# AIGC-Audio/AudioGPT

Hardware: NVIDIA H100
Metric: mel_frames_per_s_vocoded (higher is better)
Workload: dtype f32

## Files before the change

### audiogpt_b200/csrc/tapconv.cuh

```cuda
#pragma once
#include <cuda_fp16.h>
#include "common.cuh"

namespace agpt {

constexpr int kMaxTaps = 12;
constexpr int TC_BM = 128;
constexpr int TC_KC = 8;

enum Pro : int { PRO_NONE = 0, PRO_LRELU = 1, PRO_ADDVEC = 2, PRO_SILU = 3 };
enum Epi : int {
  EPI_BIAS = 0,
  EPI_RES = 1,
  EPI_ACC = 2,
  EPI_RELU = 3,
  EPI_ADDVEC = 4,
  EPI_GATE = 5,
  EPI_GEGLU = 6,
  EPI_DIFFOUT = 7,
  EPI_STORE_CF = 8,
  EPI_TANH = 9,
  EPI_MISH = 10,
  EPI_SILU = 11,
  EPI_GELU_SCALED = 12,
};

struct TapConvParams {
  const float* in; long in_gstride; int in_pitch;
  const float* w;
  const float* bias;
  float* out; long out_gstride; int out_pitch;
  int G, L, Wreal, Cin, cin_pad, Cout, cout_pad;
  int ntaps; int tap_off[kMaxTaps];
  int lo_al, R;
  int pro; float slope; const float* pvec; int pvec_gstride;
  int epi; const float* res; long res_gstride; int res_pitch; float scale; int accumulate;
  const float* evec; int evec_gstride;
  float* out2; long out2_gstride; int out2_pitch; int csplit;
  const float* w_h; const float* w_h256; const float* w_h64; const float* w_h96; int tc_chunks_h; float tc_descale;
  int tc_bn, tc_na, tc_nw, tc_nr, tc_nwk, tc_nb, tc_tps, tc_flags, tc_flags_user;
  long long* dbg;
  float flops_scale;
  int strips, strip_w;
  __half* pl_hi; __half* pl_lo; int pl_pitch;
  int tc_tall;
  const __half* pi_hi; const __half* pi_lo;
  __half* po_hi; __half* po_lo; float po_slope;
  int tc_dual;
  int tc_pipe;
  int tc_narrow_pipe;
  int tc_conv_pipe;
};

__host__ __device__ inline int tc_wv(const TapConvParams& P) { return P.Wreal > 0 ? (P.strips > 0 ? P.strip_w + 2 : P.Wreal + 1) : 0; }
__host__ __device__ inline int tc_lv(const TapConvParams& P) { const int wv = tc_wv(P); return wv ? (P.L / P.Wreal) * wv : P.L; }
__host__ __device__ inline int tc_groups(const TapConvParams& P) { return P.strips > 0 ? P.G * P.strips : P.G; }
__host__ __device__ inline int tc_sample(const TapConvParams& P, int gz) { return P.strips > 0 ? gz / P.strips : gz; }
__host__ __device__ inline int tc_row_in(const TapConvParams& P, int gz, int q, int Wv, int Lv) {
  if (q < 0 || q >= Lv) return -1;
  if (!Wv) return q;
  const int h = q / Wv, j = q - h * Wv;
  if (P.strips > 0) {
    const int w = (gz % P.strips) * P.strip_w + j - 1;
    return (w >= 0 && w < P.Wreal) ? h * P.Wreal + w : -1;
  }
  return j < P.Wreal ? h * P.Wreal + j : -1;
}
__host__ __device__ inline int tc_row_out(const TapConvParams& P, int gz, int q, int Wv, int Lv) {
  if (q < 0 || q >= Lv) return -1;
  if (!Wv) return q;
  const int h = q / Wv, j = q - h * Wv;
  if (P.strips > 0) {
    if (j < 1 || j > P.strip_w) return -1;
    const int w = (gz % P.strips) * P.strip_w + j - 1;
    return w < P.Wreal ? h * P.Wreal + w : -1;
  }
  return j < P.Wreal ? h * P.Wreal + j : -1;
}


struct PackedConv {
  DevBuf w, b, w_h, w_h256, w_h64, w_h96;
  int tc_bn = 0, h_chunks = 0;
  float h_descale = 1.f;
  int Cin = 0, cin_pad = 0, Cout = 0, cout_pad = 0, ntaps = 0;
  int tap_off_1d[kMaxTaps] = {0};
  bool is2d = false;
  bool has_bias = false;
  float useful = 1.f;
};

inline int tc_pick_bn(int cout) {
  if (cout <= 32) return 32;
  if (cout <= 64) return 64;
  const int w128 = round_up(cout, 128), w64 = round_up(cout, 64);
  return (w128 <= w64) ? 128 : 64;
}

struct PackedConv;
void tapconv_launch(TapConvParams P, cudaStream_t st);
void tcconv_launch(TapConvParams P, cudaStream_t st);
bool tcconv5_launch(TapConvParams P, cudaStream_t st);
bool tcpair_launch(TapConvParams c1, TapConvParams c2, cudaStream_t st);
struct HTile { int bn; const float* w; long ntiles; int mt; };
HTile pick_h_tile(const TapConvParams& P, int sms);
void pack_h_weights(struct PackedConv& pc, const std::vector<float>& h);
bool tcconv_supported(const TapConvParams& P);
void pack_tc_weights(struct PackedConv& pc, const std::vector<float>& h);
void tc_set_enabled(int on);
bool tc_enabled();
void profile_enable(int on);
void* profile_begin(const TapConvParams& P, bool tc, double bytes_override, cudaStream_t st);
void* profile_begin_pair(const TapConvParams& c1, const TapConvParams& c2, cudaStream_t st);
void profile_end(void* rec, cudaStream_t st);
void profile_count_tall();
long long profile_tall_launches();
void profile_count_dual();
long long profile_dual_launches();
void profile_count_pipe();
long long profile_pipe_launches();
void profile_count_narrow_pipe();
long long profile_narrow_pipe_launches();
void profile_count_conv_pipe();
long long profile_conv_pipe_launches();
void profile_count_plane();
long long profile_plane_launches();
void tapconv_note_launch(int tc, int bn, int mt, int plane);
void tapconv_last_launch(int ran[4]);
void plane_split(const float* x, __half* hi, __half* lo, long n, float slope, cudaStream_t st);
void profile_collect(double* ms, double* flops, double* bytes, long long* launches);
long profile_dump(char* out, long cap);
double fma_peak_tflops();

inline TapConvParams tapconv_params(const PackedConv& pc, int G, int L, int Wreal, int dil) {
  TapConvParams P;
  memset(&P, 0, sizeof(P));
  P.w = pc.w.p;
  P.bias = pc.has_bias ? pc.b.p : nullptr;
  P.G = G; P.L = L; P.Wreal = Wreal;
  P.Cin = pc.Cin; P.cin_pad = pc.cin_pad; P.Cout = pc.Cout; P.cout_pad = pc.cout_pad;
  P.ntaps = pc.ntaps;
  if (pc.is2d) {
    AGPT_CHECK(pc.ntaps == 9 && Wreal > 0, "2d conv needs W");
    const int Wv = Wreal + 1;
    for (int dh = -1, t = 0; dh <= 1; ++dh)
      for (int dw = -1; dw <= 1; ++dw, ++t) P.tap_off[t] = dh * Wv + dw;
  } else {
    for (int t = 0; t < pc.ntaps; ++t) P.tap_off[t] = pc.tap_off_1d[t] * dil;
  }
  P.scale = 1.f;
  P.flops_scale = pc.useful;
  P.tc_bn = pc.tc_bn;
  P.w_h = pc.w_h.p; P.w_h256 = pc.w_h256.p; P.w_h64 = pc.w_h64.p; P.w_h96 = pc.w_h96.p; P.tc_chunks_h = pc.h_chunks; P.tc_descale = pc.h_descale;
  return P;
}

inline void tapconv_set_strips(TapConvParams& P, int strip_w) {
  AGPT_CHECK(P.Wreal > 0 && P.ntaps == 9 && strip_w >= 8, "strip mode is for 3x3 convs");
  P.strips = cdiv(P.Wreal, strip_w);
  P.strip_w = strip_w;
  const int Wv = strip_w + 2;
  for (int dh = -1, t = 0; dh <= 1; ++dh)
    for (int dw = -1; dw <= 1; ++dw, ++t) P.tap_off[t] = dh * Wv + dw;
}

inline void pack_conv(PackedConv& pc, const float* w, const float* b, int Cout, int Cin, int K, bool is2d,
                      float wscale = 1.f) {
  pc.Cin = Cin; pc.Cout = Cout; pc.cin_pad = round_up(Cin, TC_KC); pc.cout_pad = round_up(Cout, 32);
  pc.ntaps = K; pc.is2d = is2d;
  std::vector<float> h((size_t)K * pc.cin_pad * pc.cout_pad, 0.f);
  for (int co = 0; co < Cout; ++co)
    for (int ci = 0; ci < Cin; ++ci)
      for (int k = 0; k < K; ++k)
        h[((size_t)k * pc.cin_pad + ci) * pc.cout_pad + co] = w[((size_t)co * Cin + ci) * K + k] * wscale;
  pc.w.upload(h);
  pack_tc_weights(pc, h);
  if (!is2d) {
    const int c = (K - 1) / 2;
    for (int k = 0; k < K; ++k) pc.tap_off_1d[k] = k - c;
  }
  pc.has_bias = b != nullptr;
  std::vector<float> hb(pc.cout_pad, 0.f);
  if (b) for (int co = 0; co < Cout; ++co) hb[co] = b[co];
  pc.b.upload(hb);
}

inline void pack_conv_grouped(PackedConv& pc, const float* w, const float* b, int C, int K, int g) {
  const int c = (K - 1) / 2;
  auto fdiv = [](int a, int d) { return a >= 0 ? a / d : -((-a + d - 1) / d); };
  const int smin = fdiv(-c, g), smax = fdiv(g - 1 + K - 1 - c, g);
  const int nt = smax - smin + 1;
  AGPT_CHECK(nt <= kMaxTaps, "grouped conv: too many super-taps");
  const int Cg = g * C;
  std::vector<float> wg((size_t)Cg * Cg * nt, 0.f), bg(Cg, 0.f);
  for (int j = 0; j < g; ++j)
    for (int co = 0; co < C; ++co) {
      if (b) bg[j * C + co] = b[co];
      for (int i = 0; i < g; ++i)
        for (int ci = 0; ci < C; ++ci)
          for (int s = smin; s <= smax; ++s) {
            const int t = g * s + i - j + c;
            if (t < 0 || t >= K) continue;
            wg[((size_t)(j * C + co) * Cg + (i * C + ci)) * nt + (s - smin)] = w[((size_t)co * C + ci) * K + t];
          }
    }
  pack_conv(pc, wg.data(), b ? bg.data() : nullptr, Cg, Cg, nt, false);
// ... 50 lines not shown
```

### audiogpt_b200/csrc/tcconv5.cu

```cuda
#include "tapconv.cuh"
#include "tapconv_epi.cuh"
#include "tc_common.cuh"
#include "tc_h16.cuh"
#include "tc_tma.cuh"
#include "models.h"

namespace agpt {

namespace {

constexpr int MAX_NA = 4, MAX_NW = 8;
constexpr int kMaxDyn = 227 * 1024 - 256;
constexpr int kDualDyn = 113 * 1024 - 256;

struct Tc5Smem {
  uint32_t a_hi[MAX_NA], a_lo[MAX_NA], w[MAX_NW], raw[2], rowinfo, rowp, bars, total;
};
__host__ __device__ inline void tc5_layout(Tc5Smem& s, int BN, int MT, int RRA, int NA, int NW, int NR, bool pl = false,
                                           int raw_pitch = 256) {
  uint32_t o = 0;
  for (int i = 0; i < MAX_NA; ++i) { s.a_hi[i] = o; if (i < NA) o += RRA * 128; }
  for (int i = 0; i < MAX_NA; ++i) { s.a_lo[i] = o; if (i < NA) o += RRA * 128; }
  for (int i = 0; i < MAX_NW; ++i) { s.w[i] = o; if (i < NW) o += 2 * BN * 128; }
  for (int i = 0; i < 2; ++i) { s.raw[i] = o; if (i < NR) o += RRA * raw_pitch; }
// ... 621 lines not shown
      if ((MT == TC_TALL || HALF) && blk == 0) load_block(0);
      named_bar_sync(1, NWK);
      const int jc = xt & 7;
      const float4 cv = epi_colvec(P2, g, cb + 4 * jc);
#pragma unroll
      for (int i = 0; i < 8; ++i) {
        const int idx = xt + i * NWK;
        const int row = (idx >> 3) & (MT - 1);
        if (pp[i] >= 0)
          epi_store_cv<PL>(P2, g, pp[i], cb + 4 * jc, *reinterpret_cast<const float4*>(stg + sw128(row, jc)), pre[i], cv);
        if (i + LA < nitem) {
          const int idxa = idx + LA * NWK;
          pp[i + LA] = rowp[item_row(xt, i + LA)];
          if (pp[i + LA] >= 0) epi_load(P2, g, pp[i + LA], cb + 4 * (idxa & 7), pre[i + LA]);
        }
      }
      if (cb + 32 < BN) load_block(cb + 32);
    }
  } else if (lane == 0) {
    const uint32_t bytes = 2u * BN * 128u;
    const int total2 = P2.tc_chunks_h * P2.ntaps;
    for (int it = 0; it < total + total2; ++it) {
      if constexpr (PL)
        if (it < total && it % P1.ntaps == 0) pl_load_chunk(smem, S, tmh, tml, a_full, a_empty, NA, it / P1.ntaps, qa + lo, g, RRA);
      const int s = it % NW, n = it / NW;
      if (n >= 1) mbar_wait(&w_empty[s], (uint32_t)((n - 1) & 1));
      mbar_arrive_expect_tx(&w_full[s], bytes);
      const uint8_t* src = it < total ? reinterpret_cast<const uint8_t*>(P1.w_h) + (size_t)it * bytes
                                      : reinterpret_cast<const uint8_t*>(P2.w_h) + (size_t)(it - total) * bytes;
      bulk_g2s(smem + S.w[s], src, bytes, &w_full[s]);
    }
  }
}

template <int BN, int MT>
__global__ void __launch_bounds__(V5_THREADS, 1) tcpair_kernel(const __grid_constant__ TapConvParams P1,
                                                               const __grid_constant__ TapConvParams P2) {
  tcpair_body<BN, MT, false>(P1, P2, nullptr, nullptr);
}
template <int BN>
__global__ void __launch_bounds__(V5_THREADS, 2) tcpair2_kernel(const __grid_constant__ TapConvParams P1,
                                                                const __grid_constant__ TapConvParams P2) {
  tcpair_body<BN, TC_ROWS, false, true>(P1, P2, nullptr, nullptr);
}
template <int BN, int MT>
__global__ void __launch_bounds__(V5_THREADS, 1) tcpair_pl_kernel(const __grid_constant__ TapConvParams P1,
                                                                 const __grid_constant__ TapConvParams P2,
                                                                 const __grid_constant__ CUtensorMap tmh,
                                                                 const __grid_constant__ CUtensorMap tml) {
  tcpair_body<BN, MT, true>(P1, P2, &tmh, &tml);
}

constexpr int PIPE_THREADS = 512;
constexpr int PIPE_MMA = 256, PIPE_DATA = 128;
template <int N> __device__ __forceinline__ void setmaxnreg_inc() { asm volatile("setmaxnreg.inc.sync.aligned.u32 %0;" ::"n"(N)); }
template <int N> __device__ __forceinline__ void setmaxnreg_dec() { asm volatile("setmaxnreg.dec.sync.aligned.u32 %0;" ::"n"(N)); }

struct PipeSmem { uint32_t set[2], w[MAX_NW], bars, total; };
__host__ __device__ inline void pipe_layout(PipeSmem& s, int R1, int NW) {
  uint32_t o = 0;
  for (int i = 0; i < 2; ++i) { s.set[i] = o; o += (uint32_t)R1 * 512; }
  for (int i = 0; i < MAX_NW; ++i) { s.w[i] = o; if (i < NW) o += 2 * 128 * 128; }
  s.bars = o; o += (2 * MAX_NW + 4) * 8;
  s.total = o;
}

__global__ void __launch_bounds__(PIPE_THREADS, 1) tcpair_pipe_kernel(const __grid_constant__ TapConvParams P1,
                                                                      const __grid_constant__ TapConvParams P2) {
  constexpr int BN = 128, MT = TC_ROWS;
  extern __shared__ uint8_t smem_raw_[];
  uint8_t* smem = reinterpret_cast<uint8_t*>((reinterpret_cast<uintptr_t>(smem_raw_) + 1023) & ~(uintptr_t)1023);
  const int R1 = P1.R, NW = P1.tc_nw;
  __shared__ PipeSmem S;
  if (threadIdx.x == 0) pipe_layout(S, R1, NW);
  __syncthreads();
  uint64_t* w_full = reinterpret_cast<uint64_t*>(smem + S.bars);
  uint64_t* w_empty = w_full + MAX_NW;
  uint64_t* in_full = w_full + 2 * MAX_NW;
  uint64_t* acc_full = in_full + 2;

  const int tid = threadIdx.x, warp = tid >> 5, lane = tid & 31;
  const int wg = __shfl_sync(0xffffffffu, tid >> 7, 0);
  int span2 = 0;
  for (int t = 0; t < P2.ntaps; ++t) span2 = max(span2, P2.tap_off[t] - P2.lo_al);
  const int Lv = P1.L, MTO = MT - span2, ntx = (Lv + MTO - 1) / MTO, ntiles = ntx * P1.G;
  const int nloc = (int)blockIdx.x < ntiles ? (ntiles - 1 - (int)blockIdx.x) / (int)gridDim.x + 1 : 0;
  const int lo = P1.lo_al, nch = P1.tc_chunks_h, total1 = nch * P1.ntaps;
  const int RR2 = P2.R, nch2 = P2.tc_chunks_h, total2 = nch2 * P2.ntaps;
  auto tile_of = [&](int k, int& g, int& q0) {
    const int T = (int)blockIdx.x + k * (int)gridDim.x;
    g = T / ntx;
    q0 = (T - g * ntx) * MTO;
  };

  if (tid == 0) {
    for (int i = 0; i < NW; ++i) { mbar_init(&w_full[i], 1); mbar_init(&w_empty[i], PIPE_MMA / 32); }
    for (int i = 0; i < 2; ++i) { mbar_init(&in_full[i], PIPE_DATA); mbar_init(&acc_full[i], PIPE_MMA); }
    fence_barrier_init();
  }
  __syncthreads();
  pdl_wait();

  if (wg < 2) {
    setmaxnreg_inc<168>();
    float acc[BN / 2];
    int it = 0, prev = -1;
    auto mma_taps = [&](const TapConvParams& Q, uint32_t ahi0, uint32_t alo0, int ksteps) {
      for (int t = 0; t < Q.ntaps; ++t, ++it) {
        const int s = it % NW;
        mbar_wait(&w_full[s], (uint32_t)((it / NW) & 1));
        const uint32_t shift = (uint32_t)Q.tap_off[t] * 128u;
        const uint64_t dah = make_desc(ahi0 + shift), dal = make_desc(alo0 + shift);
        const uint32_t ws = smem_u32(smem + S.w[s]);
        fence_acc<BN / 2>(acc);
        wgmma_fence();
        for (int k = 0; k < ksteps; ++k) {
          const uint64_t ko = (uint64_t)((k * 32) >> 4);
          const uint64_t dwh = make_desc(ws) + ko, dwl = make_desc(ws + BN * 128) + ko;
          wgmma_n128(acc, dah + ko, dwh);
          wgmma_n128(acc, dal + ko, dwh);
          wgmma_n128(acc, dah + ko, dwl);
        }
        wgmma_commit();
        wgmma_wait<1>();
        fence_acc<BN / 2>(acc);
        if (prev >= 0 && lane == 0) mbar_arrive(&w_empty[prev]);
        prev = s;
      }
    };
    auto drain = [&]() {
      wgmma_wait<0>();
      fence_acc<BN / 2>(acc);
      if (prev >= 0 && lane == 0) mbar_arrive(&w_empty[prev]);
      prev = -1;
    };
    const int r0 = wg * (MT / 2) + (warp & 3) * 16 + (lane >> 2), c0 = 2 * (lane & 3);
    for (int k = 0; k < nloc; ++k) {
      int g, q0;
      tile_of(k, g, q0);
      const int qa = q0 + P2.lo_al;
      uint8_t* set = smem + S.set[k & 1];
#pragma unroll
      for (int i = 0; i < BN / 2; ++i) acc[i] = 0.f;
      mbar_wait(&in_full[k & 1], (uint32_t)((k >> 1) & 1));
      for (int c = 0; c < nch; ++c) {
        const uint32_t ahi0 = smem_u32(set) + (uint32_t)c * R1 * 128 + (uint32_t)(wg * (MT / 2) - lo) * 128u;
        mma_taps(P1, ahi0, ahi0 + (uint32_t)nch * R1 * 128, (min(H_KCH, P1.Cin - c * H_KCH) + 15) >> 4);
      }
      drain();
      named_bar_sync(1, PIPE_MMA);
      const uint32_t lo_part = (uint32_t)nch2 * RR2 * 128;
      const float dsc1 = P1.tc_descale;
#pragma unroll
      for (int i = 0; i < BN / 8; ++i) {
        const int col = 8 * i + c0;
        const bool cok = col < P2.Cin;
        float2 bv = make_float2(0.f, 0.f);
        if (cok && P1.bias) bv = __ldg(reinterpret_cast<const float2*>(P1.bias + col));
        uint8_t* hi = set + (uint32_t)(col >> 6) * RR2 * 128;
#pragma unroll
        for (int h = 0; h < 2; ++h) {
          const int r = r0 + 8 * h;
          float v0 = 0.f, v1 = 0.f;
          if (cok && qa + r >= 0 && qa + r < Lv) {
            v0 = lrelu(__fadd_rn(__fmul_rn(acc[4 * i + 2 * h], dsc1), bv.x), P2.slope);
            v1 = lrelu(__fadd_rn(__fmul_rn(acc[4 * i + 2 * h + 1], dsc1), bv.y), P2.slope);
          }
          uint32_t l;
          const uint32_t hw = split2(v0, v1, l);
          const uint32_t o = sw128(r, (col & 63) >> 3) + (col & 7) * 2;
          *reinterpret_cast<uint32_t*>(hi + o) = hw;
          *reinterpret_cast<uint32_t*>(hi + lo_part + o) = l;
        }
      }
      const int zitems = (RR2 - MT) * 8;
      for (int idx = tid; idx < zitems * 2 * nch2; idx += PIPE_MMA) {
        const int blk = idx / zitems, u = idx - blk * zitems;
        *reinterpret_cast<uint4*>(set + (uint32_t)blk * RR2 * 128 + MT * 128 + u * 16) = make_uint4(0u, 0u, 0u, 0u);
      }
#pragma unroll
      for (int i = 0; i < BN / 2; ++i) acc[i] = 0.f;
      fence_proxy_async();
      named_bar_sync(1, PIPE_MMA);
      for (int c = 0; c < nch2; ++c) {
        const uint32_t ahi0 = smem_u32(set) + (uint32_t)c * RR2 * 128 + (uint32_t)(wg * (MT / 2) - P2.lo_al) * 128u;
        mma_taps(P2, ahi0, ahi0 + lo_part, (min(H_KCH, P2.Cin - c * H_KCH) + 15) >> 4);
      }
      drain();
      named_bar_sync(1, PIPE_MMA);
      const float dsc = P2.tc_descale;
#pragma unroll
      for (int blk = 0; blk < BN / 32; ++blk) {
        uint8_t* stg = set + blk * (MT * 128);
        const float* a = &acc[4 * (blk * 32 / 8)];
#pragma unroll
        for (int i8 = 0; i8 < 4; ++i8) {
          const int col = 8 * i8 + c0;
          *reinterpret_cast<float2*>(stg + sw128(r0, col >> 2) + (col & 3) * 4) = make_float2(a[4 * i8] * dsc, a[4 * i8 + 1] * dsc);
          *reinterpret_cast<float2*>(stg + sw128(r0 + 8, col >> 2) + (col & 3) * 4) =
              make_float2(a[4 * i8 + 2] * dsc, a[4 * i8 + 3] * dsc);
        }
      }
      mbar_arrive(&acc_full[k & 1]);
    }
  } else if (wg == 2) {
    setmaxnreg_inc<152>();
    const int dt = tid - PIPE_MMA;
    auto transform = [&](int k) {
      int g, q0;
      tile_of(k, g, q0);
      const int rin = q0 + P2.lo_al + lo;
      const float* __restrict__ ing = P1.in + g * P1.in_gstride;
      uint8_t* set = smem + S.set[k & 1];
      const int items = R1 * nch * 8;
#pragma unroll 4
      for (int idx = dt; idx < items; idx += PIPE_DATA) {
        const int row = idx / (nch * 8), c = (idx >> 3) % nch, q = idx & 7;
        const int r = rin + row, ch = c * H_KCH + 8 * q;
        float4 v0 = make_float4(0.f, 0.f, 0.f, 0.f), v1 = v0;
        if (r >= 0 && r < Lv && ch < P1.Cin) {
          v0 = ldg_stream(ing + (long)r * P1.in_pitch + ch);
          v1 = ldg_stream(ing + (long)r * P1.in_pitch + ch + 4);
        }
        const float4 x0 = pro_apply5(P1, v0, true, nullptr), x1 = pro_apply5(P1, v1, true, nullptr);
        uint4 h, l;
        h.x = split2(x0.x, x0.y, l.x);
        h.y = split2(x0.z, x0.w, l.y);
        h.z = split2(x1.x, x1.y, l.z);
        h.w = split2(x1.z, x1.w, l.w);
        const uint32_t o = (uint32_t)c * R1 * 128 + sw128(row, q);
        *reinterpret_cast<uint4*>(set + o) = h;
        *reinterpret_cast<uint4*>(set + (uint32_t)nch * R1 * 128 + o) = l;
      }
      fence_proxy_async();
      mbar_arrive(&in_full[k & 1]);
    };
    auto epilogue = [&](int k) {
      int g, q0;
      tile_of(k, g, q0);
      const uint8_t* set = smem + S.set[k & 1];
      const int jc = dt & 7;
      for (int blk = 0; blk < BN / 32; ++blk) {
        const int cb = blk * 32;
        const uint8_t* stg = set + blk * (MT * 128);
        const float4 cv = epi_colvec(P2, g, cb + 4 * jc);
        for (int h = 0; h < 2; ++h) {
          EpiPre pre[4];
          int pp[4];
#pragma unroll
          for (int i = 0; i < 4; ++i) {
            const int row = (dt + (4 * h + i) * PIPE_DATA) >> 3;
            pp[i] = (row < MTO && q0 + row < Lv) ? q0 + row : -1;
            if (pp[i] >= 0) epi_load(P2, g, pp[i], cb + 4 * jc, pre[i]);
          }
#pragma unroll
          for (int i = 0; i < 4; ++i) {
            const int row = (dt + (4 * h + i) * PIPE_DATA) >> 3;
            if (pp[i] >= 0)
              epi_store_cv(P2, g, pp[i], cb + 4 * jc, *reinterpret_cast<const float4*>(stg + sw128(row, jc)), pre[i], cv);
          }
        }
      }
    };
    if (nloc > 0) transform(0);
    for (int k = 0; k < nloc; ++k) {
      if (k + 1 < nloc) transform(k + 1);
      mbar_wait(&acc_full[k & 1], (uint32_t)((k >> 1) & 1));
      epilogue(k);
      named_bar_sync(2, PIPE_DATA);
    }
  } else {
    setmaxnreg_dec<24>();
    if (warp != 12 || lane != 0) return;
    const uint32_t bytes = 2u * BN * 128u;
    int n_it = 0;
    for (int k = 0; k < nloc; ++k)
      for (int it = 0; it < total1 + total2; ++it, ++n_it) {
        const int s = n_it % NW, n = n_it / NW;
        if (n >= 1) mbar_wait(&w_empty[s], (uint32_t)((n - 1) & 1));
        mbar_arrive_expect_tx(&w_full[s], bytes);
        const uint8_t* src = it < total1 ? reinterpret_cast<const uint8_t*>(P1.w_h) + (size_t)it * bytes
                                         : reinterpret_cast<const uint8_t*>(P2.w_h) + (size_t)(it - total1) * bytes;
        bulk_g2s(smem + S.w[s], src, bytes, &w_full[s]);
      }
  }
}

constexpr int NARROW_THREADS = 640;
constexpr int NARROW_MMA = 256, NARROW_DATA = 128, NARROW_WG = 128;
constexpr int NARROW_MMA_REGS = 112, NARROW_XF_REGS = 80, NARROW_EPI_REGS = 152;
constexpr int NARROW_MAX_NS = 4, NARROW_MAX_NW = 22;
struct NarrowSmem { uint32_t op[NARROW_MAX_NS], raw[NARROW_MAX_NS], w[NARROW_MAX_NW], bars, total; };
__host__ __device__ inline void narrow_layout(NarrowSmem& s, int BN, int R1, int nbox, int NS, int NW) {
  uint32_t o = 0;
  for (int i = 0; i < NARROW_MAX_NS; ++i) { s.op[i] = o; if (i < NS) o += (uint32_t)R1 * 256; }
  for (int i = 0; i < NARROW_MAX_NS; ++i) { s.raw[i] = o; if (i < NS) o += (uint32_t)R1 * 128 * nbox; }
  for (int i = 0; i < NARROW_MAX_NW; ++i) { s.w[i] = o; if (i < NW) o += 2u * BN * 128; }
  s.bars = o; o += (2 * NARROW_MAX_NW + 4 * NARROW_MAX_NS) * 8;
  s.total = o;
}

template <int BN>
__global__ void __launch_bounds__(NARROW_THREADS, 1) tcpair_narrow_kernel(const __grid_constant__ TapConvParams P1,
                                                                          const __grid_constant__ TapConvParams P2,
                                                                          const __grid_constant__ CUtensorMap tmx) {
  constexpr int NB = tc5_nb(BN), MT = TC_ROWS;
  static_assert(NB == BN && BN <= 64, "narrow pairs: one wgmma column block");
  extern __shared__ uint8_t smem_raw_[];
  uint8_t* smem = reinterpret_cast<uint8_t*>((reinterpret_cast<uintptr_t>(smem_raw_) + 1023) & ~(uintptr_t)1023);
  const int R1 = P1.R, NS = P1.tc_na, NW = P1.tc_nw, nbox = (P1.Cin + 31) >> 5;
  __shared__ NarrowSmem S;
  if (threadIdx.x == 0) narrow_layout(S, BN, R1, nbox, NS, NW);
  __syncthreads();
  uint64_t* w_full = reinterpret_cast<uint64_t*>(smem + S.bars);
  uint64_t* w_empty = w_full + NARROW_MAX_NW;
  uint64_t* raw_full = w_empty + NARROW_MAX_NW;
  uint64_t* in_full = raw_full + NARROW_MAX_NS;
  uint64_t* acc_full = in_full + NARROW_MAX_NS;
  uint64_t* set_free = acc_full + NARROW_MAX_NS;

  const int tid = threadIdx.x, warp = tid >> 5, lane = tid & 31;
  const int wg = __shfl_sync(0xffffffffu, tid >> 7, 0);
  int span2 = 0;
  for (int t = 0; t < P2.ntaps; ++t) span2 = max(span2, P2.tap_off[t] - P2.lo_al);
  const int Lv = P1.L, MTO = MT - span2, ntx = (Lv + MTO - 1) / MTO, ntiles = ntx * P1.G;
  const int nloc = (int)blockIdx.x < ntiles ? (ntiles - 1 - (int)blockIdx.x) / (int)gridDim.x + 1 : 0;
  const int lo = P1.lo_al, RR2 = P2.R;
  const int total1 = P1.ntaps, iters = total1 + P2.ntaps;
  const bool wres = NW == iters;
  auto tile_of = [&](int k, int& g, int& q0) {
    const int T = (int)blockIdx.x + k * (int)gridDim.x;
    g = T / ntx;
    q0 = (T - g * ntx) * MTO;
  };

  if (tid == 0) {
// ... 453 lines not shown
  const int nct = cdiv(pc.Cout, BN), nch = cdiv(pc.Cin, H_KCH), nt = pc.ntaps;
  const size_t blk = (size_t)BN * 64;
  std::vector<uint16_t> img((size_t)nct * nch * nt * 2 * blk, 0);
  for (int ct = 0; ct < nct; ++ct)
    for (int c = 0; c < nch; ++c)
      for (int t = 0; t < nt; ++t) {
        uint16_t* hi = &img[((((size_t)ct * nch + c) * nt + t) * 2) * blk];
        uint16_t* lo = hi + blk;
        for (int j = 0; j < BN; ++j) {
          const int co = ct * BN + j;
          if (co >= pc.Cout) continue;
          for (int k = 0; k < H_KCH; ++k) {
            const int ci = c * H_KCH + k;
            if (ci >= pc.Cin) continue;
            const float w = h[((size_t)t * pc.cin_pad + ci) * pc.cout_pad + co] * wscale;
            const __half wh = __float2half_rn(w);
            const __half wl = __float2half_rn(w - __half2float(wh));
            const size_t off = (size_t)j * 64 + (size_t)(((k >> 3) ^ (j & 7)) << 3) + (k & 7);
            memcpy(&hi[off], &wh, 2);
            memcpy(&lo[off], &wl, 2);
          }
        }
      }
  std::vector<float> packed((img.size() + 1) / 2, 0.f);
  memcpy(packed.data(), img.data(), img.size() * 2);
  dst.upload(packed);
}

__global__ void plane_split_kernel(const float4* __restrict__ x, uint2* __restrict__ hi, uint2* __restrict__ lo, long n4,
                                  float slope) {
  for (long i = blockIdx.x * (long)blockDim.x + threadIdx.x; i < n4; i += (long)gridDim.x * blockDim.x) {
    float4 v = x[i];
    v.x = lrelu(v.x, slope); v.y = lrelu(v.y, slope); v.z = lrelu(v.z, slope); v.w = lrelu(v.w, slope);
    uint2 h, l;
    h.x = split2(v.x, v.y, l.x);
    h.y = split2(v.z, v.w, l.y);
    hi[i] = h;
    lo[i] = l;
  }
}

}

void plane_split(const float* x, __half* hi, __half* lo, long n, float slope, cudaStream_t st) {
  AGPT_CHECK(n % 4 == 0, "plane_split: element count must be a multiple of 4");
  const long n4 = n / 4;
  const int blocks = (int)std::min<long>(cdivl(n4, 256), 132L * 16);
  plane_split_kernel<<<blocks, 256, 0, st>>>(reinterpret_cast<const float4*>(x), reinterpret_cast<uint2*>(hi),
                                             reinterpret_cast<uint2*>(lo), n4, slope);
  count_launch(1);
  AGPT_CUDA(cudaGetLastError());
}

void pack_h_weights(PackedConv& pc, const std::vector<float>& h) {
  float mx = 0.f;
  for (float v : h) mx = std::max(mx, std::fabs(v));
  int e = 0;
  float wscale = 1.f;
  if (mx > 0.f && std::isfinite(mx)) {
    std::frexp(mx, &e);
    wscale = std::ldexp(1.f, std::max(-60, std::min(60, 14 - e)));
  }
  pc.h_descale = 1.f / wscale;
  pc.h_chunks = cdiv(pc.Cin, H_KCH);
  build_h_image(pc, h, pc.tc_bn, wscale, pc.w_h);
  if (pc.tc_bn == 128) build_h_image(pc, h, 64, wscale, pc.w_h64);
  if (pc.tc_bn == 128 && pc.Cout > 128) build_h_image(pc, h, 96, wscale, pc.w_h96);
}

static int tc5_rows(TapConvParams& P, int MT) {
  int lo = P.tap_off[0], hi = P.tap_off[0];
  for (int t = 1; t < P.ntaps; ++t) { lo = std::min(lo, P.tap_off[t]); hi = std::max(hi, P.tap_off[t]); }
  P.lo_al = lo;
  P.R = round_up(MT + (hi - lo), 8);
  return hi - lo;
}

static bool tc5_plan(TapConvParams& P, int BN, int MT, long a_min, int iters, size_t& smem) {
  const int RRA = P.R;
  const bool pl = P.pi_hi != nullptr;
  P.tc_bn = BN;
  const long avail = (long)kMaxDyn - 1024  - (RRA * 4 + MT * 4 + 512) ;
  const long abytes = 2L * (pl ? pl_rows(RRA) : RRA) * 128, wbytes = 2L * BN * 128;
  const long rbytes = (long)RRA * 256;
  const long stg = 2L * MT * 128;
  const int nch = P.tc_chunks_h;
  int NA = pl ? MAX_NA : ((P.ntaps == 1) ? 3 : 2);
  NA = std::max(1, std::min(NA, nch));
  if ((long)NA * abytes < stg) NA = (int)cdiv(stg, abytes);
  int NR = pl ? 0 : ((nch > 1) ? 2 : 1);
  auto fits4 = [&](int na) { return na * abytes + 4 * wbytes <= avail; };
  while (pl && NA > 2 && !fits4(NA) && (NA - 1) * abytes >= stg) --NA;
  auto fits = [&](int na, int nr, int nw) { return na * abytes + nr * rbytes + nw * wbytes <= avail; };
  if (!fits(NA, NR, 2) && NA == 3) NA = 2;
  if (!fits(NA, NR, 2) && NR == 2) NR = 1;
  if (!fits(NA, NR, 2) && NA == 2 && abytes >= stg) NA = 1;
  if (NA * abytes < a_min) {
    NA = (int)cdiv(a_min, abytes);
    if (!fits(NA, NR, 2) && NR == 2) NR = 1;
  }
  if (NA > MAX_NA || !fits(NA, NR, 2)) return false;
  int NW = (int)std::min<long>(MAX_NW, (avail - NA * abytes - NR * rbytes) / wbytes);
  NW = std::max(2, std::min(NW, std::max(2, iters)));
  P.tc_na = NA; P.tc_nw = NW; P.tc_nr = NR;
  Tc5Smem S;
  tc5_layout(S, BN, MT, pl ? pl_rows(RRA) : RRA, NA, NW, NR, pl);
  smem = (size_t)S.total + 1024;
  return smem <= (size_t)kMaxDyn;
}

static bool tcpair_plan_dual(TapConvParams& P, int BN, long a_min, int iters, size_t& smem) {
  if (P.tc_chunks_h != 1) return false;
  const long abytes = 2L * P.R * 128, wbytes = 2L * BN * 128;
  const int NA = (int)cdiv(std::max(a_min, 2L * TC_ROWS * 128), abytes);
  if (NA > MAX_NA) return false;
  for (int NR = cdiv(P.Cin, 32); NR >= 1; --NR) {
    Tc5Smem S;
    tc5_layout(S, BN, TC_ROWS, P.R, NA, 2, NR, false, 128);
    const long spare = (long)kDualDyn - 1024 - S.total;
    if (spare < 0) continue;
// ... 113 lines not shown
  if (P.tc_bn == 128 && allow96) consider(96, P.w_h96);
  const long tall = (long)cdiv(Lv, TC_TALL) * tc_groups(P) * cdiv(P.Cout, best.bn);
  if (tc5_tall(P, best.bn, tall, sms)) { best.mt = TC_TALL; best.ntiles = tall; }
  return best;
}

static bool tcpair_try(TapConvParams P1, TapConvParams P2, int MT, bool dual, cudaStream_t st) {
  const int BN = P1.tc_bn;
  tc5_rows(P1, MT);
  const int span2 = tc5_rows(P2, MT);
  P2.tc_bn = BN;
  size_t smem = 0;
  const long a2bytes = 2L * P2.tc_chunks_h * P2.R * 128;
  const int iters = P1.tc_chunks_h * P1.ntaps + P2.tc_chunks_h * P2.ntaps;
  if (dual ? !tcpair_plan_dual(P1, BN, a2bytes, iters, smem) : !tc5_plan(P1, BN, MT, a2bytes, iters, smem)) return false;
  dim3 grid(cdiv(tc_lv(P1), MT - span2), 1, tc_groups(P1));
  tc5_set_smem_limits();
  if (dual) {
    int per_sm = 0;
    AGPT_CUDA(cudaOccupancyMaxActiveBlocksPerMultiprocessor(
        &per_sm, BN == 64 ? tcpair2_kernel<64> : tcpair2_kernel<32>, V5_THREADS, smem));
    if (per_sm != 2) return false;
  }
  void* rec = profile_begin_pair(P1, P2, st);
  tapconv_note_launch(1, BN, MT, P1.pi_hi ? 1 : 0);
  if (dual) {
    if (BN == 64) launch_pdl(tcpair2_kernel<64>, grid, dim3(V5_THREADS), smem, st, P1, P2);
    else launch_pdl(tcpair2_kernel<32>, grid, dim3(V5_THREADS), smem, st, P1, P2);
    profile_count_dual();
  } else if (P1.pi_hi) {
    const PlMaps m = pl_tensor_maps(P1);
    if (MT == TC_TALL) {
      if (BN == 64) launch_pdl(tcpair_pl_kernel<64, TC_TALL>, grid, dim3(V5_THREADS), smem, st, P1, P2, m.hi, m.lo);
      else launch_pdl(tcpair_pl_kernel<32, TC_TALL>, grid, dim3(V5_THREADS), smem, st, P1, P2, m.hi, m.lo);
      profile_count_tall();
    } else if (BN == 128) launch_pdl(tcpair_pl_kernel<128, TC_ROWS>, grid, dim3(V5_THREADS), smem, st, P1, P2, m.hi, m.lo);
    else if (BN == 64) launch_pdl(tcpair_pl_kernel<64, TC_ROWS>, grid, dim3(V5_THREADS), smem, st, P1, P2, m.hi, m.lo);
    else launch_pdl(tcpair_pl_kernel<32, TC_ROWS>, grid, dim3(V5_THREADS), smem, st, P1, P2, m.hi, m.lo);
    profile_count_plane();
  } else if (MT == TC_TALL) {
    if (BN == 64) launch_pdl(tcpair_kernel<64, TC_TALL>, grid, dim3(V5_THREADS), smem, st, P1, P2);
    else launch_pdl(tcpair_kernel<32, TC_TALL>, grid, dim3(V5_THREADS), smem, st, P1, P2);
    profile_count_tall();
  } else if (BN == 128) launch_pdl(tcpair_kernel<128, TC_ROWS>, grid, dim3(V5_THREADS), smem, st, P1, P2);
  else if (BN == 64) launch_pdl(tcpair_kernel<64, TC_ROWS>, grid, dim3(V5_THREADS), smem, st, P1, P2);
  else launch_pdl(tcpair_kernel<32, TC_ROWS>, grid, dim3(V5_THREADS), smem, st, P1, P2);
  profile_end(rec, st);
  count_launch(1);
  AGPT_CUDA(cudaGetLastError());
  return true;
}

static bool tcpair_pipe_try(TapConvParams P1, TapConvParams P2, cudaStream_t st) {
  if (!P1.tc_pipe || P1.tc_bn != 128 || P1.Cin != 128 || P1.Cout != 128 || P2.Cout != 128 || P1.pi_hi || P2.po_hi)
    return false;
  tc5_rows(P1, TC_ROWS);
  const int span2 = tc5_rows(P2, TC_ROWS);
  if (P2.R > P1.R) return false;
  const long wbytes = 2L * 128 * 128;
  PipeSmem S;
  pipe_layout(S, P1.R, 0);
  const long spare = (long)kMaxDyn - 1024 - (long)S.total;
  if (spare < 2 * wbytes) return false;
  const int iters = P1.tc_chunks_h * P1.ntaps + P2.tc_chunks_h * P2.ntaps;
  P1.tc_nw = (int)std::min<long>(std::min<long>(MAX_NW, std::max(2, iters)), spare / wbytes);
  P2.tc_bn = 128;
  pipe_layout(S, P1.R, P1.tc_nw);
  const size_t smem = (size_t)S.total + 1024;
  const long tiles = (long)cdiv(P1.L, TC_ROWS - span2) * P1.G;
  dim3 grid((unsigned)std::min<long>(tiles, tc5_sms()));
  int dev = 0;
  AGPT_CUDA(cudaGetDevice(&dev));
  static bool attr_done_dev[64] = {false};
  if (!attr_done_dev[dev & 63]) {
    AGPT_CUDA(cudaFuncSetAttribute(tcpair_pipe_kernel, cudaFuncAttributeMaxDynamicSharedMemorySize, kMaxDyn));
    attr_done_dev[dev & 63] = true;
  }
  void* rec = profile_begin_pair(P1, P2, st);
  tapconv_note_launch(1, 128, TC_ROWS, 0);
  launch_pdl(tcpair_pipe_kernel, grid, dim3(PIPE_THREADS), smem, st, P1, P2);
  profile_count_pipe();
  profile_end(rec, st);
  count_launch(1);
  AGPT_CUDA(cudaGetLastError());
  return true;
}

static bool tcpair_dual(const TapConvParams& P1) {
  return P1.tc_dual && P1.tc_bn <= 64 && !P1.pi_hi;
}

static bool tcpair_narrow_try(TapConvParams P1, TapConvParams P2, cudaStream_t st) {
  const int BN = P1.tc_bn, iters = P1.ntaps + P2.ntaps;
  if (!P1.tc_narrow_pipe || (BN != 64 && BN != 32) || (BN == 64 && iters > 14) || P1.Cin > BN || P2.po_hi ||
      P2.res != P1.in || P2.res_pitch != P1.in_pitch || P2.res_gstride != P1.in_gstride)
    return false;
  const int span1 = tc5_rows(P1, TC_ROWS);
  const int span2 = tc5_rows(P2, TC_ROWS);
  if (P2.R > P1.R || P1.R > 256 || P1.lo_al > 0 || P2.lo_al > 0 || (P1.lo_al + span1) + (P2.lo_al + span2) < 0)
    return false;
  const int nbox = cdiv(P1.Cin, 32);
  const long wbytes = 2L * BN * 128, set = 256L * P1.R + 128L * nbox * P1.R;
  NarrowSmem S;
  narrow_layout(S, BN, P1.R, nbox, 0, 0);
  const long avail = (long)kMaxDyn - 1024 - (long)S.total;
  int NS = 2, NW;
  if (avail - iters * wbytes >= 2 * set) {
    NW = iters;
    NS = (int)std::min<long>(NARROW_MAX_NS, (avail - iters * wbytes) / set);
  } else {
    NW = (int)std::min<long>(iters, (avail - NS * set) / wbytes);
    if (NW < 2) return false;
  }
  CUtensorMap tmx;
  if (!tma_encode_rows(&tmx, P1.in, P1.Cin, P1.L, P1.G, P1.in_pitch, P1.in_gstride, P1.R)) return false;
  P1.tc_na = NS; P1.tc_nw = NW;
  P2.tc_bn = BN;
  narrow_layout(S, BN, P1.R, nbox, NS, NW);
// ... 87 lines not shown
```

Measured before the change: 200,800.

## Split pipe-kernel weight stages into half-K 64-channel chunks with separate image

```diff
diff --git a/audiogpt_b200/csrc/tapconv.cuh b/audiogpt_b200/csrc/tapconv.cuh
--- a/audiogpt_b200/csrc/tapconv.cuh
+++ b/audiogpt_b200/csrc/tapconv.cuh
@@ -38,6 +38,7 @@
   const float* evec; int evec_gstride;
   float* out2; long out2_gstride; int out2_pitch; int csplit;
   const float* w_h; const float* w_h256; const float* w_h64; const float* w_h96; int tc_chunks_h; float tc_descale;
+  const float* w_hk;
   int tc_bn, tc_na, tc_nw, tc_nr, tc_nwk, tc_nb, tc_tps, tc_flags, tc_flags_user;
   long long* dbg;
   float flops_scale;
@@ -80,7 +81,7 @@
 
 
 struct PackedConv {
-  DevBuf w, b, w_h, w_h256, w_h64, w_h96;
+  DevBuf w, b, w_h, w_h256, w_h64, w_h96, w_hk;
   int tc_bn = 0, h_chunks = 0;
   float h_descale = 1.f;
   int Cin = 0, cin_pad = 0, Cout = 0, cout_pad = 0, ntaps = 0;
@@ -151,7 +152,7 @@
   P.scale = 1.f;
   P.flops_scale = pc.useful;
   P.tc_bn = pc.tc_bn;
-  P.w_h = pc.w_h.p; P.w_h256 = pc.w_h256.p; P.w_h64 = pc.w_h64.p; P.w_h96 = pc.w_h96.p; P.tc_chunks_h = pc.h_chunks; P.tc_descale = pc.h_descale;
+  P.w_h = pc.w_h.p; P.w_h256 = pc.w_h256.p; P.w_h64 = pc.w_h64.p; P.w_h96 = pc.w_h96.p; P.w_hk = pc.w_hk.p; P.tc_chunks_h = pc.h_chunks; P.tc_descale = pc.h_descale;
   return P;
 }
 
diff --git a/audiogpt_b200/csrc/tcconv5.cu b/audiogpt_b200/csrc/tcconv5.cu
--- a/audiogpt_b200/csrc/tcconv5.cu
+++ b/audiogpt_b200/csrc/tcconv5.cu
@@ -697,16 +697,26 @@
 }
 
 constexpr int PIPE_THREADS = 512;
+constexpr uint32_t PIPE_STAGE = 2u * 128u * 64u;
+__device__ __forceinline__ uint64_t make_desc64(uint32_t saddr) {
+  uint64_t d = 0;
+  d |= (uint64_t)((saddr & 0x3FFFF) >> 4);
+  d |= (uint64_t)1 << 16;
+  d |= (uint64_t)(512 >> 4) << 32;
+  d |= (uint64_t)2 << 62;
+  return d;
+}
 constexpr int PIPE_MMA = 256, PIPE_DATA = 128;
 template <int N> __device__ __forceinline__ void setmaxnreg_inc() { asm volatile("setmaxnreg.inc.sync.aligned.u32 %0;" ::"n"(N)); }
 template <int N> __device__ __forceinline__ void setmaxnreg_dec() { asm volatile("setmaxnreg.dec.sync.aligned.u32 %0;" ::"n"(N)); }
 
-struct PipeSmem { uint32_t set[2], w[MAX_NW], bars, total; };
+constexpr int PIPE_MAX_NW = 8;
+struct PipeSmem { uint32_t set[2], w[PIPE_MAX_NW], bars, total; };
 __host__ __device__ inline void pipe_layout(PipeSmem& s, int R1, int NW) {
   uint32_t o = 0;
   for (int i = 0; i < 2; ++i) { s.set[i] = o; o += (uint32_t)R1 * 512; }
-  for (int i = 0; i < MAX_NW; ++i) { s.w[i] = o; if (i < NW) o += 2 * 128 * 128; }
-  s.bars = o; o += (2 * MAX_NW + 4) * 8;
+  for (int i = 0; i < PIPE_MAX_NW; ++i) { s.w[i] = o; if (i < NW) o += PIPE_STAGE; }
+  s.bars = o; o += (2 * PIPE_MAX_NW + 4) * 8;
   s.total = o;
 }
 
@@ -720,8 +730,8 @@
   if (threadIdx.x == 0) pipe_layout(S, R1, NW);
   __syncthreads();
   uint64_t* w_full = reinterpret_cast<uint64_t*>(smem + S.bars);
-  uint64_t* w_empty = w_full + MAX_NW;
-  uint64_t* in_full = w_full + 2 * MAX_NW;
+  uint64_t* w_empty = w_full + PIPE_MAX_NW;
+  uint64_t* in_full = w_full + 2 * PIPE_MAX_NW;
   uint64_t* acc_full = in_full + 2;
 
   const int tid = threadIdx.x, warp = tid >> 5, lane = tid & 31;
@@ -730,8 +740,8 @@
   for (int t = 0; t < P2.ntaps; ++t) span2 = max(span2, P2.tap_off[t] - P2.lo_al);
   const int Lv = P1.L, MTO = MT - span2, ntx = (Lv + MTO - 1) / MTO, ntiles = ntx * P1.G;
   const int nloc = (int)blockIdx.x < ntiles ? (ntiles - 1 - (int)blockIdx.x) / (int)gridDim.x + 1 : 0;
-  const int lo = P1.lo_al, nch = P1.tc_chunks_h, total1 = nch * P1.ntaps;
-  const int RR2 = P2.R, nch2 = P2.tc_chunks_h, total2 = nch2 * P2.ntaps;
+  const int lo = P1.lo_al, nch = P1.tc_chunks_h, total1 = 2 * nch * P1.ntaps;
+  const int RR2 = P2.R, nch2 = P2.tc_chunks_h, total2 = 2 * nch2 * P2.ntaps;
   auto tile_of = [&](int k, int& g, int& q0) {
     const int T = (int)blockIdx.x + k * (int)gridDim.x;
     g = T / ntx;
@@ -750,28 +760,30 @@
     setmaxnreg_inc<168>();
     float acc[BN / 2];
     int it = 0, prev = -1;
-    auto mma_taps = [&](const TapConvParams& Q, uint32_t ahi0, uint32_t alo0, int ksteps) {
-      for (int t = 0; t < Q.ntaps; ++t, ++it) {
-        const int s = it % NW;
-        mbar_wait(&w_full[s], (uint32_t)((it / NW) & 1));
-        const uint32_t shift = (uint32_t)Q.tap_off[t] * 128u;
-        const uint64_t dah = make_desc(ahi0 + shift), dal = make_desc(alo0 + shift);
-        const uint32_t ws = smem_u32(smem + S.w[s]);
-        fence_acc<BN / 2>(acc);
-        wgmma_fence();
-        for (int k = 0; k < ksteps; ++k) {
-          const uint64_t ko = (uint64_t)((k * 32) >> 4);
-          const uint64_t dwh = make_desc(ws) + ko, dwl = make_desc(ws + BN * 128) + ko;
-          wgmma_n128(acc, dah + ko, dwh);
-          wgmma_n128(acc, dal + ko, dwh);
-          wgmma_n128(acc, dah + ko, dwl);
-        }
-        wgmma_commit();
-        wgmma_wait<1>();
-        fence_acc<BN / 2>(acc);
-        if (prev >= 0 && lane == 0) mbar_arrive(&w_empty[prev]);
-        prev = s;
-      }
+    auto mma_taps = [&](const TapConvParams& Q, uint32_t ahi0, uint32_t alo0) {
+      for (int t = 0; t < Q.ntaps; ++t)
+        for (int hf = 0; hf < 2; ++hf, ++it) {
+          const int s = it % NW;
+          mbar_wait(&w_full[s], (uint32_t)((it / NW) & 1));
+          const uint32_t shift = (uint32_t)Q.tap_off[t] * 128u;
+          const uint64_t dah = make_desc(ahi0 + shift) + 4 * hf, dal = make_desc(alo0 + shift) + 4 * hf;
+          const uint32_t ws = smem_u32(smem + S.w[s]);
+          fence_acc<BN / 2>(acc);
+          wgmma_fence();
+#pragma unroll
+          for (int k = 0; k < 2; ++k) {
+            const uint64_t ko = (uint64_t)((k * 32) >> 4);
+            const uint64_t dwh = make_desc64(ws) + ko, dwl = make_desc64(ws + BN * 64) + ko;
+            wgmma_n128(acc, dah + ko, dwh);
+            wgmma_n128(acc, dal + ko, dwh);
+            wgmma_n128(acc, dah + ko, dwl);
+          }
+          wgmma_commit();
+          wgmma_wait<1>();
+          fence_acc<BN / 2>(acc);
+          if (prev >= 0 && lane == 0) mbar_arrive(&w_empty[prev]);
+          prev = s;
+        }
     };
     auto drain = [&]() {
       wgmma_wait<0>();
@@ -790,7 +802,7 @@
       mbar_wait(&in_full[k & 1], (uint32_t)((k >> 1) & 1));
       for (int c = 0; c < nch; ++c) {
         const uint32_t ahi0 = smem_u32(set) + (uint32_t)c * R1 * 128 + (uint32_t)(wg * (MT / 2) - lo) * 128u;
-        mma_taps(P1, ahi0, ahi0 + (uint32_t)nch * R1 * 128, (min(H_KCH, P1.Cin - c * H_KCH) + 15) >> 4);
+        mma_taps(P1, ahi0, ahi0 + (uint32_t)nch * R1 * 128);
       }
       drain();
       named_bar_sync(1, PIPE_MMA);
@@ -829,7 +841,7 @@
       named_bar_sync(1, PIPE_MMA);
       for (int c = 0; c < nch2; ++c) {
         const uint32_t ahi0 = smem_u32(set) + (uint32_t)c * RR2 * 128 + (uint32_t)(wg * (MT / 2) - P2.lo_al) * 128u;
-        mma_taps(P2, ahi0, ahi0 + lo_part, (min(H_KCH, P2.Cin - c * H_KCH) + 15) >> 4);
+        mma_taps(P2, ahi0, ahi0 + lo_part);
       }
       drain();
       named_bar_sync(1, PIPE_MMA);
@@ -917,16 +929,15 @@
   } else {
     setmaxnreg_dec<24>();
     if (warp != 12 || lane != 0) return;
-    const uint32_t bytes = 2u * BN * 128u;
     int n_it = 0;
     for (int k = 0; k < nloc; ++k)
       for (int it = 0; it < total1 + total2; ++it, ++n_it) {
         const int s = n_it % NW, n = n_it / NW;
         if (n >= 1) mbar_wait(&w_empty[s], (uint32_t)((n - 1) & 1));
-        mbar_arrive_expect_tx(&w_full[s], bytes);
-        const uint8_t* src = it < total1 ? reinterpret_cast<const uint8_t*>(P1.w_h) + (size_t)it * bytes
-                                         : reinterpret_cast<const uint8_t*>(P2.w_h) + (size_t)(it - total1) * bytes;
-        bulk_g2s(smem + S.w[s], src, bytes, &w_full[s]);
+        mbar_arrive_expect_tx(&w_full[s], PIPE_STAGE);
+        const uint8_t* src = it < total1 ? reinterpret_cast<const uint8_t*>(P1.w_hk) + (size_t)it * PIPE_STAGE
+                                         : reinterpret_cast<const uint8_t*>(P2.w_hk) + (size_t)(it - total1) * PIPE_STAGE;
+        bulk_g2s(smem + S.w[s], src, PIPE_STAGE, &w_full[s]);
       }
   }
 }
@@ -1486,6 +1497,31 @@
   AGPT_CUDA(cudaGetLastError());
 }
 
+static void build_hk_image(const PackedConv& pc, const std::vector<float>& h, float wscale, DevBuf& dst) {
+  const int nch = cdiv(pc.Cin, H_KCH), nt = pc.ntaps;
+  const size_t blk = (size_t)128 * 32;
+  std::vector<uint16_t> img((size_t)nch * nt * 2 * 2 * blk, 0);
+  for (int c = 0; c < nch; ++c)
+    for (int t = 0; t < nt; ++t)
+      for (int hf = 0; hf < 2; ++hf) {
+        uint16_t* hi = &img[((((size_t)c * nt + t) * 2 + hf) * 2) * blk];
+        uint16_t* lo = hi + blk;
+        for (int j = 0; j < 128; ++j)
+          for (int k = 0; k < 32; ++k) {
+            const int ci = c * H_KCH + hf * 32 + k;
+            const float w = h[((size_t)t * pc.cin_pad + ci) * pc.cout_pad + j] * wscale;
+            const __half wh = __float2half_rn(w);
+            const __half wl = __float2half_rn(w - __half2float(wh));
+            const size_t off = (size_t)j * 32 + (size_t)(((k >> 3) ^ ((j >> 1) & 3)) << 3) + (k & 7);
+            memcpy(&hi[off], &wh, 2);
+            memcpy(&lo[off], &wl, 2);
+          }
+      }
+  std::vector<float> packed((img.size() + 1) / 2, 0.f);
+  memcpy(packed.data(), img.data(), img.size() * 2);
+  dst.upload(packed);
+}
+
 void pack_h_weights(PackedConv& pc, const std::vector<float>& h) {
   float mx = 0.f;
   for (float v : h) mx = std::max(mx, std::fabs(v));
@@ -1500,6 +1536,7 @@
   build_h_image(pc, h, pc.tc_bn, wscale, pc.w_h);
   if (pc.tc_bn == 128) build_h_image(pc, h, 64, wscale, pc.w_h64);
   if (pc.tc_bn == 128 && pc.Cout > 128) build_h_image(pc, h, 96, wscale, pc.w_h96);
+  if (pc.tc_bn == 128 && pc.Cin == 128 && pc.Cout == 128 && !pc.is2d) build_hk_image(pc, h, wscale, pc.w_hk);
 }
 
 static int tc5_rows(TapConvParams& P, int MT) {
@@ -1719,18 +1756,19 @@
 }
 
 static bool tcpair_pipe_try(TapConvParams P1, TapConvParams P2, cudaStream_t st) {
-  if (!P1.tc_pipe || P1.tc_bn != 128 || P1.Cin != 128 || P1.Cout != 128 || P2.Cout != 128 || P1.pi_hi || P2.po_hi)
+  if (!P1.tc_pipe || P1.tc_bn != 128 || P1.Cin != 128 || P1.Cout != 128 || P2.Cout != 128 || P1.pi_hi || P2.po_hi ||
+      !P1.w_hk || !P2.w_hk)
     return false;
   tc5_rows(P1, TC_ROWS);
   const int span2 = tc5_rows(P2, TC_ROWS);
   if (P2.R > P1.R) return false;
-  const long wbytes = 2L * 128 * 128;
+  const long wbytes = PIPE_STAGE;
   PipeSmem S;
   pipe_layout(S, P1.R, 0);
   const long spare = (long)kMaxDyn - 1024 - (long)S.total;
-  if (spare < 2 * wbytes) return false;
-  const int iters = P1.tc_chunks_h * P1.ntaps + P2.tc_chunks_h * P2.ntaps;
-  P1.tc_nw = (int)std::min<long>(std::min<long>(MAX_NW, std::max(2, iters)), spare / wbytes);
+  if (spare < 4 * wbytes) return false;
+  const int iters = 2 * (P1.tc_chunks_h * P1.ntaps + P2.tc_chunks_h * P2.ntaps);
+  P1.tc_nw = (int)std::min<long>(std::min<long>(PIPE_MAX_NW, iters), spare / wbytes);
   P2.tc_bn = 128;
   pipe_layout(S, P1.R, P1.tc_nw);
   const size_t smem = (size_t)S.total + 1024;
```

Result: faster. 212,300, median of 6 (+5.7%).
